# netty/netty

Measured on AMD Instinct MI355X. Metric: GiB/s device-resident Snappy encode+decode, 64 KiB chunks, 1/2/4/8 MI355X, higher is better.
Workload: dtype u8; 1 GPU; configs[4]: Snappy encode (+frame CRC32C) then decode + CRC32C verify of 1638400 text-like 64 KiB chunks (100 GiB) split across 1 GPU(s), device-resident; chunk_bytes=65536, global_chunks=1638400, chunks_per_gpu=1638400, parallelism=dp1 (independent chunk shards, no data-path collective)

## Files before the change

### netty_amd/csrc/snappy_decode.hip

```cpp
#include <stddef.h>
#include <stdlib.h>
#include <type_traits>
#include <string.h>
#include <algorithm>
#include <map>
#include <mutex>
#include "nx_common.hpp"
#include "workspace.hpp"
#include "records.hpp"

namespace nx {
namespace dec {

constexpr int kWaves = 12;
#ifndef NX_RING
#define NX_RING 2048
#endif
constexpr int kRing = NX_RING;
constexpr int kStage = 1024;
constexpr int kFB = 512;
constexpr int kPass = 256;
static_assert((kRing & (kRing - 1)) == 0 && kRing >= 3 * kFB + kPass + 2, "ring");
constexpr int32_t kGuardTrip = -99;
constexpr uint32_t kRecCap = 16384;
constexpr int32_t kNeedFused = -1000;
constexpr uint32_t kSubBatch = NX_DEC_MAX_FRAMES;
constexpr uint32_t kFusedMaxFrames = 32768;
constexpr int kDecodeAuto = 0, kDecodeFused = 1, kDecodePair = 2;

constexpr int kTabWords = 4 * 256 + 4 * 256;
constexpr int kTabBytes = kTabWords * 4;

struct WaveLds {
    uint32_t ring[kRing / 4];
    uint32_t tagw[2 * 64 + 2];
    uint32_t scratch[65];
    uint32_t pad[1];
    uint32_t stage[kStage / 4];
};
constexpr uint32_t kStageDw = offsetof(WaveLds, stage) / 4;
static_assert(sizeof(WaveLds) % 16 == 0 && offsetof(WaveLds, stage) % 16 == 0, "keep per-wave LDS 16-byte aligned");
static_assert(2 * (kTabBytes + kWaves * sizeof(WaveLds)) <= 160 * 1024, "two workgroups per CU");

#ifndef NX_EXPAND_STAGE
#define NX_EXPAND_STAGE 0
#endif
constexpr bool kExpandStaged = NX_EXPAND_STAGE != 0;
constexpr size_t kExpandWaveLds = kExpandStaged ? sizeof(WaveLds) : offsetof(WaveLds, stage);
#ifndef NX_EXPAND_WAVES
#define NX_EXPAND_WAVES (NX_EXPAND_STAGE ? 12 : 4)
#endif
constexpr int kExpandWaves = NX_EXPAND_WAVES;
#ifndef NX_EXPAND_MINB
#define NX_EXPAND_MINB (NX_EXPAND_STAGE ? 3 : 8)
#endif
static_assert(kTabBytes + kExpandWaves * kExpandWaveLds <= 160 * 1024 / NX_EXPAND_MINB, "k_expand workgroups per CU");

typedef uint32_t __attribute__((aligned(1))) u32u;
typedef __attribute__((address_space(1))) const uint8_t gu8;
typedef __attribute__((address_space(1))) const u32u gu32u;
typedef unsigned int v4u __attribute__((ext_vector_type(4)));
typedef __attribute__((address_space(1))) const v4u gv4u;

__device__ __forceinline__ uint32_t shift_byte_tab(const uint32_t* __restrict__ S, uint32_t c) {
    return S[c & 0xFF] ^ S[256 + ((c >> 8) & 0xFF)] ^ S[512 + ((c >> 16) & 0xFF)] ^ S[768 + (c >> 24)];
}

__device__ __forceinline__ uint32_t shift_nib_tab(const uint32_t* __restrict__ N, uint32_t c) {
    uint32_t r = 0;
#pragma unroll
    for (int k = 0; k < 8; ++k) r ^= N[k * 16 + ((c >> (4 * k)) & 15u)];
    return r;
}

__device__ __forceinline__ uint32_t raw8(const uint32_t* __restrict__ T, uint32_t w0, uint32_t w1) {
    uint32_t c = w0;
    c = T[3 * 256 + (c & 0xFF)] ^ T[2 * 256 + ((c >> 8) & 0xFF)] ^ T[1 * 256 + ((c >> 16) & 0xFF)] ^ T[c >> 24];
    c ^= w1;
    c = T[3 * 256 + (c & 0xFF)] ^ T[2 * 256 + ((c >> 8) & 0xFF)] ^ T[1 * 256 + ((c >> 16) & 0xFF)] ^ T[c >> 24];
    return c;
}

__device__ __forceinline__ uint32_t uni(uint32_t v) { return (uint32_t)__builtin_amdgcn_readfirstlane((int)v); }

__device__ __forceinline__ void wave_sync() {
    __builtin_amdgcn_fence(__ATOMIC_RELEASE, "wavefront");
    __builtin_amdgcn_wave_barrier();
    __builtin_amdgcn_fence(__ATOMIC_ACQUIRE, "wavefront");
}

__device__ __forceinline__ uint64_t lanemask_le(int lane) { return lane == 63 ? ~0ull : ((2ull << lane) - 1ull); }

__device__ __forceinline__ uint32_t incl_scan(uint32_t v) {
    v += (uint32_t)__builtin_amdgcn_update_dpp(0, (int)v, 0x111, 0xf, 0xf, false);
    v += (uint32_t)__builtin_amdgcn_update_dpp(0, (int)v, 0x112, 0xf, 0xf, false);
    v += (uint32_t)__builtin_amdgcn_update_dpp(0, (int)v, 0x114, 0xf, 0xf, false);
    v += (uint32_t)__builtin_amdgcn_update_dpp(0, (int)v, 0x118, 0xf, 0xf, false);
    v += (uint32_t)__builtin_amdgcn_update_dpp(0, (int)v, 0x142, 0xa, 0xf, false);
    v += (uint32_t)__builtin_amdgcn_update_dpp(0, (int)v, 0x143, 0xc, 0xf, false);
    return v;
}

__device__ __forceinline__ uint32_t incl_max_scan(uint32_t v) {
    v = max(v, (uint32_t)__builtin_amdgcn_update_dpp(0, (int)v, 0x111, 0xf, 0xf, false));
    v = max(v, (uint32_t)__builtin_amdgcn_update_dpp(0, (int)v, 0x112, 0xf, 0xf, false));
    v = max(v, (uint32_t)__builtin_amdgcn_update_dpp(0, (int)v, 0x114, 0xf, 0xf, false));
    v = max(v, (uint32_t)__builtin_amdgcn_update_dpp(0, (int)v, 0x118, 0xf, 0xf, false));
    v = max(v, (uint32_t)__builtin_amdgcn_update_dpp(0, (int)v, 0x142, 0xa, 0xf, false));
    v = max(v, (uint32_t)__builtin_amdgcn_update_dpp(0, (int)v, 0x143, 0xc, 0xf, false));
    return v;
}

__device__ __forceinline__ uint32_t g_ld32u(const uint8_t* p) { return *(gu32u*)(p); }
__device__ __forceinline__ uint32_t g_ld8(const uint8_t* p) { return *(gu8*)(p); }

struct Frame {
    const uint8_t* src;
    uint32_t in_len;
    uint8_t* dst;
    uint32_t cap;
};

struct FrameIO {
    WaveLds& L;
    const uint8_t* __restrict__ src;
    uint8_t* __restrict__ dst;
    const uint32_t* __restrict__ sT;
    const uint32_t* __restrict__ sSH;
    uint32_t in_len;
    uint32_t a;
    uint32_t aend;
    uint32_t sbase;
    uint2 pf;
    uint32_t flushed;
    uint32_t acc;
    bool dst8, do_crc;
    int lane;

    __device__ __forceinline__ FrameIO(WaveLds& L_, const Frame& f, const uint32_t* T, const uint32_t* SH, bool crc, int ln)
        : L(L_), src(f.src), dst(f.dst), sT(T), sSH(SH), in_len(uni(f.in_len)), sbase(0), pf(make_uint2(0, 0)), flushed(0),
          acc(0), do_crc(crc), lane(ln) {
        a = (uint32_t)((uintptr_t)src & 7u);
        aend = a + in_len;
        dst8 = (((uintptr_t)dst) & 7u) == 0;
    }
    __device__ __forceinline__ uint2 load8(uint32_t apos) const {
        return apos < aend ? *reinterpret_cast<const uint2*>(src - a + apos) : make_uint2(0, 0);
    }
    __device__ __forceinline__ void put8(uint32_t apos, uint2 v) {
        *reinterpret_cast<uint2*>(&reinterpret_cast<uint8_t*>(L.stage)[apos & (kStage - 1)]) = v;
    }
    __device__ __forceinline__ void prime(uint32_t wa) {
        sbase = wa & ~511u;
        put8(sbase + 8u * lane, load8(sbase + 8u * lane));
        put8(sbase + 512u + 8u * lane, load8(sbase + 512u + 8u * lane));
        pf = load8(sbase + 1024u + 8u * lane);
    }
    __device__ __forceinline__ void advance(uint32_t wa) {
        while (wa >= sbase + 512u) {
            if (wa >= sbase + 1536u) {
                prime(wa);
                break;
            }
            put8(sbase + 1024u + 8u * lane, pf);
            sbase += 512u;
            pf = load8(sbase + 1024u + 8u * lane);
        }
    }
    __device__ __forceinline__ void flush_to(uint32_t limit) {
        const uint8_t* ring8 = reinterpret_cast<const uint8_t*>(L.ring);
        while (flushed + (uint32_t)kFB <= limit) {
            wave_sync();
            asm volatile("s_waitcnt vmcnt(1)" ::: "memory");
            const uint2 d = *reinterpret_cast<const uint2*>(&ring8[(flushed + 8u * lane) & (kRing - 1)]);
            uint8_t* o = dst + flushed + 8u * lane;
            if (dst8) {
                *reinterpret_cast<uint2*>(o) = d;
            } else {
#pragma unroll
                for (int i = 0; i < 8; ++i) o[i] = (uint8_t)((i < 4 ? d.x : d.y) >> (8 * (i & 3)));
            }
            if (do_crc) acc = shift_byte_tab(sSH, acc) ^ raw8(sT, (flushed == 0u && lane == 0) ? ~d.x : d.x, d.y);
            flushed += (uint32_t)kFB;
        }
    }
    __device__ uint32_t finish(uint32_t O, const uint32_t* __restrict__ gNS) {
        const uint8_t* ring8 = reinterpret_cast<const uint8_t*>(L.ring);
        flush_to(O);
        wave_sync();
        const uint32_t rem = O - flushed;
        const uint32_t k = rem >> 3;
        asm volatile("s_waitcnt vmcnt(0)" ::: "memory");
        {
            const uint32_t b0 = 8u * lane, b1 = b0 + 8u < rem ? b0 + 8u : rem;
            for (uint32_t i = b0; i < b1; ++i) dst[flushed + i] = ring8[(flushed + i) & (kRing - 1)];
        }
        uint32_t crc = 0;
        if (do_crc) {
            auto fold = [&](uint32_t v) {
#pragma unroll
                for (int j = 0; j < 6; ++j) {
                    const uint32_t other = __shfl_xor(v, 1 << j);
                    const bool is_lo = ((lane >> j) & 1) == 0;
                    v = shift_nib_tab(gNS + j * 128, is_lo ? v : other) ^ (is_lo ? other : v);
                }
                return v;
            };
            uint32_t R = fold(acc);
            uint32_t c2 = 0;
            if ((uint32_t)lane >= 64u - k) {
                const uint32_t pos = flushed + 8u * ((uint32_t)lane - (64u - k));
                const uint2 d = *reinterpret_cast<const uint2*>(&ring8[pos & (kRing - 1)]);
                c2 = raw8(sT, pos == 0u ? ~d.x : d.x, d.y);
            }
            c2 = fold(c2);
#pragma unroll
            for (int j = 0; j < 6; ++j)
                if ((k >> j) & 1u) R = shift_nib_tab(gNS + j * 128, R);
            R ^= c2;
            if (O < 8u) R = 0xFFFFFFFFu;
            for (uint32_t i = flushed + 8u * k; i < O; ++i) R = (R >> 8) ^ sT[(R ^ ring8[i & (kRing - 1)]) & 0xFFu];
            crc = ~R;
        }
        return crc;
    }
};

struct Window {
    uint32_t rec, pdone, O;
};

__device__ bool expand_tags(FrameIO& io, uint32_t lds_base, uint32_t O, uint32_t E, bool prod, uint64_t prodm, uint32_t ostart,
                            uint32_t xv, int lane, uint32_t P0s = 0u, bool last = true, Window* nw = nullptr, uint32_t* rn = nullptr,
                            bool staged = true) {
    WaveLds& L = io.L;
    const uint8_t* ring8 = reinterpret_cast<const uint8_t*>(L.ring);
    const uint32_t* lds32 = L.ring;
    const uint32_t rank = __builtin_amdgcn_mbcnt_hi((uint32_t)(prodm >> 32), __builtin_amdgcn_mbcnt_lo((uint32_t)prodm, 0u));
    if (prod) *reinterpret_cast<uint2*>(&L.tagw[2 * rank]) = make_uint2(ostart, xv);
    if (lane == 0) L.tagw[2 * (uint32_t)__popcll(prodm)] = E;
    const uint64_t unal = __ballot(prod && (ostart & 3u) != 0u);
    const uint64_t first_bit = prodm & (~prodm + 1ull);
    const uint32_t pbase = (ostart >> 2) - (O >> 2) + (uint32_t)__popcll(unal & lanemask_le(lane) & ~first_bit);
    const uint32_t Ptot = ((E + 3u) >> 2) - (O >> 2) + (uint32_t)__popcll(unal & ~first_bit);
    uint32_t rc = 0;
    uint32_t pbc = 0;
    const uint32_t Pend = last ? Ptot : P0s + ((Ptot - P0s) & ~63u);
    uint32_t* const marks = L.scratch;
    uint32_t P0 = P0s;
    if (P0 >= Pend) {
        if (rn) asm volatile("" : "+v"(*rn));
    } else do {
        L.scratch[lane] = 0u;
        wave_sync();
        {
            const uint32_t rel = pbase - P0;
            const bool in_pass = prod && rel < 64u;
            marks[in_pass ? rel : 64u] = ((rank + 1u) << 6) | (rel & 63u);
        }
        wave_sync();
        const uint32_t mk = incl_max_scan(L.scratch[lane]);
        const uint32_t P = P0 + lane;
        const bool valid = P < Ptot;
        uint32_t r = mk ? (mk >> 6) - 1u : rc;
        const uint32_t k = mk ? (uint32_t)lane - (mk & 63u) : P - pbc;
        r = valid ? r : 0u;
        {
            const uint32_t mlast = uni((uint32_t)__builtin_amdgcn_readlane((int)mk, 63));
            if (mlast) {
                rc = (mlast >> 6) - 1u;
                pbc = P0 + (mlast & 63u);
            }
        }
        const uint32_t tstart = L.tagw[2 * r], tx = L.tagw[2 * r + 1], tend = L.tagw[2 * r + 2];
        const uint32_t A = ((tstart >> 2) + k) << 2;
        const uint32_t x0 = A > tstart ? A : tstart;
        const uint32_t x1 = (A + 4u) < tend ? A + 4u : tend;
        const uint32_t last = (Ptot - P0) < 64u ? (Ptot - P0 - 1u) : 63u;
        const uint32_t ps = uni((uint32_t)__builtin_amdgcn_readlane((int)x0, 0));
        const uint32_t pe = uni((uint32_t)__builtin_amdgcn_readlane((int)x1, (int)last));

        const bool lit = (tx & 0x80000000u) == 0u;
        const uint32_t xo = tx & 0x7FFFFFFFu;
        const uint32_t tlen = tend - tstart;
        const bool overlap = !lit && xo < tlen;
        const uint32_t pin = xo + (x0 - tstart);
        const uint32_t sp = lit ? pin + io.a : x0 - xo;
        const bool gl = lit ? (!staged || (sp - io.sbase) > (uint32_t)(kStage - 8))
                            : (!overlap && pe > (uint32_t)kRing && sp < pe - (uint32_t)kRing);
        const uint32_t lbase = lit && staged ? kStageDw : 0u;
        const uint32_t lmask = lit && staged ? (uint32_t)(kStage / 4 - 1) : (uint32_t)(kRing / 4 - 1);
        const uint32_t nbytes = x1 - x0;
        const uint32_t sh = 8u * (x0 & 3u);
        const uint32_t bmask = (nbytes >= 4u ? 0xFFFFFFFFu : ((1u << (8u * nbytes)) - 1u)) << sh;
        const uint32_t waddr = lds_base + 4u * ((x0 >> 2) & (kRing / 4 - 1));
        uint32_t gval;
        uint32_t gsh = 0;
        uint32_t gtiny = 0;
        const bool gld = valid && gl;
        const bool tiny = io.in_len < 4u;
        if (__ballot(gld)) {
            const bool tail = lit && pin + 4u > io.in_len;
            const uint8_t* ga = !lit ? io.dst + sp : io.src + (tail ? io.in_len - 4u : pin);
            if (gld && !tiny) gval = g_ld32u(ga);
            gsh = tail ? 8u * (pin + 4u - io.in_len) : 0u;
            if (tiny && __ballot(gld)) {
                if (gld) {
#pragma unroll
                    for (uint32_t i = 0; i < 4; ++i)
                        if (pin + i < io.in_len) gtiny |= g_ld8(io.src + pin + i) << (8 * i);
                }
            }
        }
        const uint32_t psal = ps & ~3u;
        const uint32_t dhi = overlap ? tstart : sp + nbytes;
        const bool dep = valid && !lit && !gl && dhi > ps;
        uint64_t need = 0;
        const uint64_t depm = __ballot(dep);
        if (depm) {
            wave_sync();
            {
                const uint32_t mm = valid ? bmask : 0u;
                const uint32_t maddr = lds_base + (uint32_t)offsetof(WaveLds, scratch) + (valid ? 4u * ((x0 >> 2) - (psal >> 2)) : 0u);
                asm volatile("ds_mskor_b32 %0, %1, %2" ::"v"(maddr), "v"(mm), "v"(((uint32_t)lane * 0x01010101u) & mm) : "memory");
            }
            wave_sync();
            const uint32_t lo0 = overlap ? tstart - xo : sp;
            const uint8_t* M8 = reinterpret_cast<const uint8_t*>(L.scratch);
            const uint32_t lo = lo0 > ps ? lo0 : ps;
            const uint32_t pa = M8[dep ? lo - psal : 0u], pb = M8[dep ? dhi - 1u - psal : 0u];
            const uint64_t nm = (pb >= 63u ? ~0ull : ((2ull << pb) - 1ull)) & ~((1ull << (pa & 63u)) - 1ull);
            need = dep ? nm : 0ull;
        }
        const bool has_ov = __ballot(valid && overlap) != 0ull;
        uint32_t ova = 0, ovb = 0;
        if (has_ov) {
            const uint32_t n0 = x0 - tstart;
            const uint32_t inv = (uint32_t)(__builtin_amdgcn_rcpf((float)xo) * 65536.0f) + 1u;
            const uint32_t m0 = n0 - xo * ((n0 * inv) >> 16);
            const uint32_t q = tstart - xo;
            uint32_t ad[4];
            uint32_t mi = m0;
#pragma unroll
            for (uint32_t i = 0; i < 4; ++i) {
                if (i) mi = mi + 1u == xo ? 0u : mi + 1u;
                ad[i] = (q + mi) & (kRing - 1);
            }
            ova = ad[0] | (ad[1] << 16);
            ovb = ad[2] | (ad[3] << 16);
        }
        const uint32_t w = sp >> 2;
        const uint32_t ra0 = lbase + (w & lmask), ra1 = lbase + ((w + 1u) & lmask);
        uint64_t pending = depm;
        const uint64_t validm = last >= 63u ? ~0ull : ((2ull << last) - 1ull);
        uint64_t readym = validm & ~depm;
        for (int round = 0;; ++round) {
            uint32_t lo = lds32[ra0];
            uint32_t hi = lds32[ra1];
            asm volatile("" : "+v"(lo), "+v"(hi));
            uint32_t val = gl ? (tiny ? gtiny : gval >> gsh) : __builtin_amdgcn_alignbyte(hi, lo, sp & 3u);
            if (has_ov) {
                const uint32_t ov = (uint32_t)ring8[ova & 0xFFFFu] | ((uint32_t)ring8[ova >> 16] << 8) |
                                    ((uint32_t)ring8[ovb & 0xFFFFu] << 16) | ((uint32_t)ring8[ovb >> 16] << 24);
                val = overlap ? ov : val;
            }
            uint32_t m;
            asm volatile("v_cndmask_b32_e64 %0, 0, %1, %2" : "=v"(m) : "v"(bmask), "s"(readym));
            asm volatile("ds_mskor_b32 %0, %1, %2" ::"v"(waddr), "v"(m), "v"((val << sh) & m) : "memory");
            if (!pending || round >= 64) break;
            readym = __ballot((need & pending) == 0ull) & validm;
            pending &= ~readym;
        }
        if (pending) return false;
        if (rn) asm volatile("" : "+v"(*rn));
        io.flush_to(pe);
    } while ((P0 += 64u) < Pend);
    if (!last) {
        if (Pend == Ptot) {
            nw->rec = (uint32_t)__popcll(prodm);
            nw->pdone = 0u;
            nw->O = E;
        } else {
            const uint32_t idx = (uint32_t)__popcll(__ballot(prod && pbase <= Pend)) - 1u;
            nw->rec = idx;
            nw->pdone = Pend - uni((uint32_t)__builtin_amdgcn_readlane((int)pbase, (int)idx));
            nw->O = uni((uint32_t)__builtin_amdgcn_readlane((int)ostart, (int)idx));
        }
    }
    return true;
}

__device__ __forceinline__ void write_result(int lane, uint32_t crc, int32_t st, bool check, uint32_t expect, uint32_t O,
                                             uint32_t consumed, uint32_t* out_len_p, uint32_t* consumed_p, int32_t* status_p,
                                             uint32_t* crc_p) {
    if (lane == 0) {
        const uint32_t m = mask_checksum(crc);
        if (st == NX_OK && check && m != expect) st = NX_ERR_SNAPPY_CRC_MISMATCH;
        *out_len_p = O;
        if (consumed_p) *consumed_p = consumed;
        *status_p = st;
        if (crc_p) *crc_p = m;
    }
}

__device__ void decode_frame_fused(WaveLds& L, uint32_t lds_base, const Frame& f, const uint32_t* __restrict__ sT,
                                   const uint32_t* __restrict__ sSH, const uint32_t* __restrict__ gNS, bool do_crc, uint32_t expect,
                                   bool check, uint32_t* out_len_p, uint32_t* consumed_p, int32_t* status_p, uint32_t* crc_p,
                                   int lane) {
    FrameIO io(L, f, sT, sSH, do_crc, lane);
    const uint8_t* __restrict__ src = f.src;
    const uint32_t in_len = io.in_len;
    const uint32_t cap = uni(f.cap < (1u << 24) ? f.cap : (1u << 24));
    int32_t st = NX_OK;
    uint32_t consumed = 0;
    uint32_t O = 0;

    uint32_t W = 0;
    bool go = false;
    if (in_len > 0) {
        uint32_t ulen = 0;
        int bi = 0;
        bool complete = false;
        while (W < in_len) {
            const uint32_t cur = uni(src[W++]);
            ulen |= (cur & 0x7fu) << (bi++ * 7);
            if ((cur & 0x80u) == 0) {
                complete = true;
                break;
            }
            if (bi >= 4) {
                st = NX_ERR_SNAPPY_PREAMBLE_TOO_LONG;
                break;
            }
        }
        if (st == NX_OK && complete && ulen != 0) {
            if (ulen > cap) st = NX_ERR_SNAPPY_OUTPUT_OVERFLOW; else go = true;
        }
        consumed = W;
    }
    W = uni(W);
    if (go) io.prime(W + io.a);

    bool stop = !go;
    uint32_t windows = 0;
    while (!stop && W < in_len) {
        if (++windows > in_len + 2) {
            st = kGuardTrip;
            break;
        }
        io.advance(W + io.a);
        wave_sync();
        const uint32_t p = W + lane;
        const uint32_t avail = p < in_len ? in_len - p : 0u;
        uint64_t v;
        {
            const uint32_t pa = p + io.a;
            const uint32_t w0 = L.stage[(pa >> 2) & (kStage / 4 - 1)];
            const uint32_t w1 = L.stage[((pa >> 2) + 1) & (kStage / 4 - 1)];
            v = (((uint64_t)w1 << 32) | w0) >> (8 * (pa & 3u));
            if (avail < 5) v &= (1ull << (8 * avail)) - 1ull;
        }
        const uint32_t b0 = (uint32_t)v & 0xFFu;
        const uint32_t type = b0 & 3u;
        const uint32_t ops = (uint32_t)(v >> 8);
        const uint32_t code = b0 >> 2;
        const uint32_t nb = code >= 60u ? code - 59u : 0u;
        const uint32_t hdr = 1u + nb;
        const uint32_t field = nb == 0 ? 0u : (nb == 4 ? ops : (ops & ((1u << (8 * nb)) - 1u)));
        const uint32_t lj = nb == 0 ? code + 1u : field + 1u;
        const bool lneg = nb == 4 && (int32_t)lj < 0;
        const bool lhdr_nei = avail < hdr;
        const bool l_nei = lhdr_nei || (!lneg && (avail - hdr) < lj);
        const uint32_t csize = type == 1u ? 2u : (type == 2u ? 3u : 5u);
        const uint32_t colen = type == 1u ? 4u + ((b0 >> 2) & 7u) : 1u + (b0 >> 2);
        const uint32_t coff = type == 1u ? (((b0 & 0xe0u) << 3) | (ops & 0xFFu)) : (type == 2u ? (ops & 0xFFFFu) : ops);
        const bool c_nei = avail < csize;
        const bool is_copy = type != 0u;
        const bool nei = is_copy ? c_nei : l_nei;
        int32_t err = 0;
        if (is_copy) {
            if (!c_nei && coff == 0u) err = NX_ERR_SNAPPY_OFFSET_ZERO;
            else if (!c_nei && type == 3u && (int32_t)coff < 0) err = NX_ERR_SNAPPY_OFFSET_NEGATIVE;
        } else if (!lhdr_nei && lneg) {
            err = NX_ERR_SNAPPY_LITERAL_LEN_INVALID;
        }
        uint32_t size;
        uint32_t olen;
        if (is_copy) {
            size = csize;
            olen = colen;
        } else {
            const uint64_t sz = (uint64_t)hdr + (lneg ? 0ull : (uint64_t)lj);
            size = sz > 0x7FFFFFFFull ? 0x7FFFFFFFu : (uint32_t)sz;
            olen = lneg ? 0u : (lj > cap ? cap + 1u : lj);
        }
        const uint32_t xv = is_copy ? (0x80000000u | (coff & 0x7FFFFFFFu)) : ((p + hdr) & 0x7FFFFFFFu);
        const uint32_t nxt = (uint32_t)lane + size;

        const uint32_t lim = uni((in_len - W) < 64u ? (in_len - W) : 64u);
        uint32_t Jk[6];
        Jk[0] = (uint32_t)lane >= lim ? (uint32_t)lane : (nxt < 64u ? nxt : 64u);
#pragma unroll
        for (int k = 1; k < 6; ++k) {
            const uint32_t prev = Jk[k - 1];
            const uint32_t g = (uint32_t)__shfl((int)prev, (int)(prev & 63u));
            Jk[k] = prev >= 64u ? 64u : g;
        }
        uint32_t pos = 0;
#pragma unroll
        for (int k = 0; k < 6; ++k) {
            const uint32_t g = (uint32_t)__shfl((int)Jk[k], (int)(pos & 63u));
            if (((uint32_t)lane >> k) & 1u) pos = pos >= 64u ? 64u : g;
        }
        const bool tvm = pos < lim;
        const uint32_t T = (uint32_t)__popcll(__ballot(tvm));
        const uint32_t lastpos = uni((uint32_t)__builtin_amdgcn_readlane((int)pos, (int)(T - 1)));
        const uint32_t exitrel = uni((uint32_t)__builtin_amdgcn_readlane((int)nxt, (int)lastpos));
        L.scratch[lane] = 0;
        wave_sync();
        if (tvm) L.scratch[pos] = 1u;
        wave_sync();
        const bool tv = L.scratch[lane] != 0u;

        const uint32_t mylen = tv ? olen : 0u;
        const uint32_t incl = incl_scan(mylen);
        const uint32_t ostart = O + incl - mylen;
        if (tv && is_copy && !nei && err == 0 && (coff & 0x7FFFFFFFu) > ostart) err = NX_ERR_SNAPPY_OFFSET_BEYOND;
        if (tv && !nei && err == 0 && (uint64_t)ostart + olen > cap) err = NX_ERR_SNAPPY_OUTPUT_OVERFLOW;
        const uint64_t badm = __ballot(tv && (nei || err != 0));
        const uint32_t Wnext = uni(W + exitrel);
        uint32_t fb = 64;
        uint32_t E;
        if (badm) {
            fb = (uint32_t)(__ffsll((long long)badm) - 1);
            const int32_t e = __builtin_amdgcn_readlane(err, (int)fb);
            if (e != 0) {
                st = e;
                consumed = W + uni((uint32_t)__builtin_amdgcn_readlane((int)nxt, (int)fb));
            } else {
                consumed = W + fb + 1;
            }
            stop = true;
            E = uni((uint32_t)__builtin_amdgcn_readlane((int)ostart, (int)fb));
        } else {
            consumed = Wnext < in_len ? Wnext : in_len;
            E = O + uni((uint32_t)__builtin_amdgcn_readlane((int)incl, 63));
        }
        const bool prod = tv && (uint32_t)lane < fb && olen > 0;
        const uint64_t prodm = __ballot(prod);
        if (prodm && !expand_tags(io, lds_base, O, E, prod, prodm, ostart, xv, lane)) {
            st = kGuardTrip + 2;
            break;
        }
        O = E;
        W = Wnext;
    }
    const uint32_t crc = io.finish(O, gNS);
    write_result(lane, crc, st, check, expect, O, consumed, out_len_p, consumed_p, status_p, crc_p);
}

struct WaveSetup {
    uint32_t* sT;
    uint32_t* sSH;
    WaveLds* L;
    uint32_t lds_base;
    uint32_t wave;
};
__device__ __forceinline__ WaveSetup wave_setup(uint8_t* smem, const CrcTables* __restrict__ tabs, bool do_crc,
                                                size_t wave_lds = sizeof(WaveLds)) {
    WaveSetup s;
    s.sT = reinterpret_cast<uint32_t*>(smem);
    s.sSH = s.sT + 4 * 256;
    if (do_crc) {
        for (int i = threadIdx.x; i < 4 * 256; i += blockDim.x) s.sT[i] = (&tabs->T8[0][0])[i];
        for (int i = threadIdx.x; i < 4 * 256; i += blockDim.x) s.sSH[i] = (&tabs->SH[5][0][0])[i];
    }
    __syncthreads();
    s.wave = uni(threadIdx.x >> 6);
    s.L = reinterpret_cast<WaveLds*>(smem + kTabBytes + s.wave * wave_lds);
    s.lds_base = (uint32_t)(uintptr_t)s.L;
    return s;
}

__global__ void __launch_bounds__(kWaves * 64, 6)
    k_decode_fused(const uint8_t* __restrict__ in, const uint64_t* __restrict__ in_off, const uint32_t* __restrict__ in_len,
                   uint8_t* __restrict__ out, const uint64_t* __restrict__ out_off, const uint32_t* __restrict__ out_cap,
// ... 98 lines not shown
            x[0].y = w[33];
            x[0].z = w[34];
            x[0].w = w[35];
        } else if (B != 0u) {
            x[0] = *(const gv4u*)(origin + (B - 16u <= last ? B - 16u : last));
        } else {
            x[0] = v4u{0u, 0u, 0u, 0u};
        }
        lb = B;
#pragma unroll
        for (uint32_t k = 0; k < 9; ++k) {
            w[4 * k] = x[k].x;
            w[4 * k + 1] = x[k].y;
            w[4 * k + 2] = x[k].z;
            w[4 * k + 3] = x[k].w;
        }
    }
    __device__ __forceinline__ uint64_t get8(uint32_t p) const {
        const uint32_t off = p + pad + 16u - lb;
        const uint32_t i = off >> 2, s = off & 3u;
        const uint32_t d0 = w[i], d1 = w[i + 1], d2 = w[i + 2];
        return (uint64_t)__builtin_amdgcn_alignbyte(d1, d0, s) | ((uint64_t)__builtin_amdgcn_alignbyte(d2, d1, s) << 32);
    }
};
#ifndef NX_PARSE_LINE
#define NX_PARSE_LINE 0
#endif
#ifndef NX_PARSE_DEFER
#define NX_PARSE_DEFER 0
#endif
#ifndef NX_PARSE_RELOAD_K
#define NX_PARSE_RELOAD_K 16
#endif


template <uint32_t QR, bool DEFER = false>
struct RecWriterT {
    static_assert(QR == 4 || QR == 8 || QR == 16, "record row");
    static constexpr uint32_t kStride = QR == 16 ? 20u : QR + 1u;
    static constexpr uint32_t kV = QR / 4;
    uint4* slot;
    uint32_t* q;
    uint32_t n;
    v4u p0, p1, p2, p3;
    uint32_t pend_at;
    __device__ __forceinline__ RecWriterT(uint4* s, uint32_t* row) : slot(s), q(row), n(0), pend_at(0xFFFFFFFFu) {}
    __device__ __forceinline__ v4u row(uint32_t k) const {
        if constexpr (QR == 16) {
            return reinterpret_cast<const v4u*>(q)[k];
        } else {
            return v4u{q[4 * k], q[4 * k + 1], q[4 * k + 2], q[4 * k + 3]};
        }
    }
    __device__ __forceinline__ void drain() {
        if constexpr (DEFER) {
            if (pend_at != 0xFFFFFFFFu) {
                v4u* d = reinterpret_cast<v4u*>(slot + (pend_at >> 2));
                d[0] = p0;
                if constexpr (kV > 1) d[1] = p1;
                if constexpr (kV > 2) {
                    d[2] = p2;
                    d[3] = p3;
                }
                pend_at = 0xFFFFFFFFu;
            }
        }
    }
    __device__ __forceinline__ bool put(uint32_t r) {
        if constexpr (!DEFER) {
            const bool ok = n < kRecCap;
            q[n & (QR - 1u)] = r;
            if (ok & ((n & (QR - 1u)) == QR - 1u)) {
                v4u* d = reinterpret_cast<v4u*>(slot + ((n - (QR - 1u)) >> 2));
#pragma unroll
                for (uint32_t k = 0; k < kV; ++k) d[k] = row(k);
            }
            n += ok ? 1u : 0u;
            return ok;
        }
        if (n >= kRecCap) return false;
        drain();
        q[n & (QR - 1u)] = r;
        if ((n & (QR - 1u)) == QR - 1u) {
            if constexpr (DEFER) {
                p0 = row(0);
                if constexpr (kV > 1) p1 = row(1);
                if constexpr (kV > 2) {
                    p2 = row(2);
                    p3 = row(3);
                }
                pend_at = n - (QR - 1u);
            } else {
                v4u* d = reinterpret_cast<v4u*>(slot + ((n - (QR - 1u)) >> 2));
#pragma unroll
                for (uint32_t k = 0; k < kV; ++k) d[k] = row(k);
            }
        }
        ++n;
        return true;
    }
    __device__ __forceinline__ void finish() {
        drain();
        const uint32_t k = n & (QR - 1u);
        if (k) {
            v4u* d = reinterpret_cast<v4u*>(slot + ((n - k) >> 2));
#pragma unroll
            for (uint32_t j = 0; j < kV; ++j)
                if (4u * j < k) d[j] = row(j);
        }
    }
};
using RecWriter = RecWriterT<16>;
constexpr int kQDw = (int)RecWriter::kStride;
#ifndef NX_PARSE_QR
#define NX_PARSE_QR 16
#endif
#ifndef NX_PARSE_NB
#define NX_PARSE_NB 4
#endif
using ParseRec = RecWriterT<NX_PARSE_QR, NX_PARSE_DEFER != 0>;
using ParseBurst = BurstWinT<NX_PARSE_NB>;
using ParseWin = std::conditional_t<NX_PARSE_LINE != 0, BurstWinLine, ParseBurst>;

template <int K, class Has, class Step>
__device__ __forceinline__ void burst_steps(const bool& run, Has has, Step step) {
    if constexpr (K > 0) {
        for (;;) {
            const bool act = run & has();
            if (!__any(act) || __popcll(__ballot(run & !act)) >= K) break;
            if (act) step();
        }
    } else {
        while (run & has()) step();
    }
}
#ifndef NX_ALT_RELOAD_K
#define NX_ALT_RELOAD_K 0
#endif

__global__ void __launch_bounds__(kParseBlock) k_parse(const uint8_t* __restrict__ in, const uint64_t* __restrict__ in_off,
                                                       const uint32_t* __restrict__ in_len_a, const uint32_t* __restrict__ out_cap,
                                                       uint32_t* __restrict__ rec, uint32_t* __restrict__ nrec,
                                                       uint32_t* __restrict__ out_len, uint32_t* __restrict__ consumed_a,
                                                       int32_t* __restrict__ status, uint32_t n, uint32_t* __restrict__ need_fused) {
    __shared__ uint32_t wins[kParseBlock * ParseWin::kStride + 4];
    __shared__ __attribute__((aligned(16))) uint32_t recq[kParseBlock * ParseRec::kStride];
    const uint32_t c = blockIdx.x * blockDim.x + threadIdx.x;
    if (c >= n) return;
    const uint32_t in_len = in_len_a[c];
    uint32_t cap = out_cap ? out_cap[c] : 65536u;
    cap = cap < (1u << 24) ? cap : (1u << 24);
    if (in_len >= (1u << 25)) {
        status[c] = kNeedFused;
        if (need_fused) *need_fused = 1u;
        return;
    }
    ParseWin win;
    win.init(in + in_off[c], in_len, &wins[threadIdx.x * ParseWin::kStride]);
    ParseRec rw(reinterpret_cast<uint4*>(rec + (size_t)c * kRecCap), &recq[threadIdx.x * ParseRec::kStride]);
    uint32_t ip = 0, op = 0;
    int32_t st = NX_OK;
    bool run = false;
    if (in_len > 0) {
        win.load(0);
        const uint64_t v = win.get8(0);
        uint32_t ulen = 0;
        int bi = 0;
        bool complete = false;
        while (ip < in_len) {
            const uint32_t cur = (uint32_t)(v >> (8 * ip)) & 0xFFu;
            ++ip;
            ulen |= (cur & 0x7fu) << (bi++ * 7);
            if ((cur & 0x80u) == 0) {
                complete = true;
                break;
            }
            if (bi >= 4) {
                st = NX_ERR_SNAPPY_PREAMBLE_TOO_LONG;
                break;
            }
        }
        if (st == NX_OK && complete && ulen != 0) {
            if (ulen > cap) st = NX_ERR_SNAPPY_OUTPUT_OVERFLOW; else run = true;
        }
    }
    auto step = [&]() {
        const uint64_t v = win.get8(ip);
        const uint32_t tag = (uint32_t)v & 0xFFu;
        const uint32_t ops = (uint32_t)(v >> 8);
        const uint32_t after_tag = ip + 1u;
        const uint32_t avail = in_len - after_tag;
        const uint32_t type = tag & 3u;
        const bool isl = type == 0u;
        const uint32_t code = tag >> 2;
        const uint32_t nb = (isl && code >= 60u) ? code - 59u : 0u;
        const uint32_t fmask = nb >= 4u ? 0xFFFFFFFFu : ((1u << (8u * nb)) - 1u);
        const uint32_t lj = nb == 0u ? code + 1u : (ops & fmask) + 1u;
        const uint32_t csize = type == 1u ? 1u : (type == 2u ? 2u : 4u);
        const uint32_t clen = type == 1u ? 4u + (code & 7u) : 1u + code;
        const uint32_t coff = type == 1u ? (((tag & 0xe0u) << 3) | (ops & 0xFFu)) : (type == 2u ? (ops & 0xFFFFu) : ops);
        const uint32_t hdr = isl ? nb : csize;
        const uint32_t dpos = after_tag + hdr;
        const bool lneg = isl && (int32_t)lj < 0;
        const bool nei = avail < hdr || (isl && !lneg && in_len - dpos < lj);
        const uint32_t len = isl ? lj : clen;
        const bool bad = (uint32_t)(isl ? lneg : coff - 1u >= op) | (uint32_t)(len > cap - op);
        if (nei | bad) {
            const int32_t cerr = coff == 0u ? NX_ERR_SNAPPY_OFFSET_ZERO
                                            : ((int32_t)coff < 0 ? NX_ERR_SNAPPY_OFFSET_NEGATIVE : (coff > op ? NX_ERR_SNAPPY_OFFSET_BEYOND : 0));
            const int32_t terr = isl ? (lneg ? NX_ERR_SNAPPY_LITERAL_LEN_INVALID : 0) : cerr;
            ip = nei ? after_tag : dpos;
            st = nei ? NX_OK : (terr != 0 ? terr : NX_ERR_SNAPPY_OUTPUT_OVERFLOW);
            run = false;
            return;
        }
        const uint32_t m0 = lj < 64u ? lj : 64u;
        const uint32_t r = isl ? (((m0 - 1u) << 25) | dpos) : (0x80000000u | ((clen - 1u) << 25) | coff);
        bool fit = (isl && lj == 0u) || rw.put(r);
        if (isl && lj > 64u) {
            for (uint32_t k = 64u; k < lj && fit; k += 64u) {
                const uint32_t m = lj - k < 64u ? lj - k : 64u;
                fit = rw.put(((m - 1u) << 25) | (dpos + k));
            }
        }
        if (!fit) {
            st = kNeedFused;
            run = false;
            return;
        }
        ip = dpos + (isl ? lj : 0u);
        op += len;
        run = ip < in_len;
    };
    for (;;) {
        run = run && ip < in_len;
        if (!__any(run)) break;
        if (run && !win.has(ip)) win.load(ip);
        burst_steps<NX_PARSE_RELOAD_K>(run, [&] { return win.has(ip); }, step);
    }
    if (st == kNeedFused) {
        status[c] = kNeedFused;
        if (need_fused) *need_fused = 1u;
        return;
    }
    rw.finish();
    nrec[c] = rw.n;
    out_len[c] = op;
    if (consumed_a) consumed_a[c] = ip;
    status[c] = st;
}

#ifdef NX_EXPAND_NUM_SGPR
#define NX_EXPAND_SGPR_ATTR __attribute__((amdgpu_num_sgpr(NX_EXPAND_NUM_SGPR)))
#else
#define NX_EXPAND_SGPR_ATTR
#endif
__global__ void __launch_bounds__(kExpandWaves * 64, NX_EXPAND_MINB) NX_EXPAND_SGPR_ATTR
    k_expand(const uint8_t* __restrict__ in, const uint64_t* __restrict__ in_off, const uint32_t* __restrict__ in_len,
             uint8_t* __restrict__ out, const uint64_t* __restrict__ out_off, const uint32_t* __restrict__ rec,
             const uint32_t* __restrict__ nrec, uint32_t* __restrict__ out_len, int32_t* __restrict__ status,
             const uint32_t* __restrict__ expect, uint32_t* __restrict__ crc_out, uint32_t n, const CrcTables* __restrict__ tabs) {
    extern __shared__ __attribute__((aligned(16))) uint8_t smem[];
    const bool do_crc = (expect != nullptr) || (crc_out != nullptr);
    const WaveSetup s = wave_setup(smem, tabs, do_crc, kExpandWaveLds);
    const int lane = threadIdx.x & 63;
    const uint32_t nw = gridDim.x * kExpandWaves;
    for (uint32_t c = blockIdx.x * kExpandWaves + s.wave; c < n; c += nw) {
        int32_t st = (int32_t)uni((uint32_t)status[c]);
        if (st == kNeedFused) continue;
        const uint32_t N = uni(nrec[c]);
        const uint32_t Ofin = uni(out_len[c]);
        Frame f{in + in_off[c], in_len[c], out + out_off[c], 0u};
        FrameIO io(*s.L, f, s.sT, s.sSH, do_crc, lane);
        const uint32_t* __restrict__ R = rec + (size_t)c * kRecCap;
        uint32_t O = 0;
        uint32_t pdone = 0;
        bool primed = false;
        uint32_t r = (uint32_t)lane < N ? R[lane] : 0u;
        asm volatile("" : "+v"(r));
        for (uint32_t b = 0; b < N;) {
            const bool valid = b + (uint32_t)lane < N;
            const bool isc = (r >> 31) != 0u;
            const uint32_t len = valid ? ((r >> 25) & 63u) + 1u : 0u;
            asm volatile("" ::"v"(len) : "memory");
            uint32_t rnext = b + 64u + (uint32_t)lane < N ? R[b + 64u + lane] : 0u;
            const uint32_t x = r & 0x1FFFFFFu;
            const uint32_t incl = incl_scan(len);
            const uint32_t ostart = O + incl - len;
            const uint32_t E = O + uni((uint32_t)__builtin_amdgcn_readlane((int)incl, 63));
            const uint64_t litm = kExpandStaged ? __ballot(valid && !isc) : 0ull;
            if (litm) {
                const uint32_t w = uni((uint32_t)__builtin_amdgcn_readlane((int)x, __ffsll((long long)litm) - 1));
                if (!primed) {
                    io.prime(w + io.a);
                    primed = true;
                } else {
                    io.advance(w + io.a);
                }
                wave_sync();
            }
            const uint32_t xv = isc ? (0x80000000u | x) : x;
            const bool last = b + 64u >= N;
            Window nw{0u, 0u, 0u};
            if (!expand_tags(io, s.lds_base, O, E, valid, __ballot(valid), ostart, xv, lane, pdone, last, &nw, &rnext, kExpandStaged)) {
                st = kGuardTrip + 2;
                break;
            }
            if (last) {
                O = E;
                break;
            }
            const uint32_t src = (uint32_t)lane + nw.rec;
            const uint32_t from_r = (uint32_t)__shfl((int)r, (int)(src & 63u));
            const uint32_t from_n = (uint32_t)__shfl((int)rnext, (int)(src & 63u));
            r = src < 64u ? from_r : from_n;
            b += nw.rec;
            pdone = nw.pdone;
            O = nw.O;
        }
        if (st == kGuardTrip + 2) O = Ofin;
        const uint32_t crc = io.finish(O, &tabs->NS[0][0][0]);
        write_result(lane, crc, st, expect != nullptr, expect ? expect[c] : 0u, O, 0u, &out_len[c], nullptr, &status[c],
                     crc_out ? &crc_out[c] : nullptr);
    }
}





__device__ __forceinline__ bool put_copy(RecWriter& rw, uint32_t len, uint32_t dist) {
    bool fit = true;
    for (uint32_t k = 0; k < len && fit; k += 64u) {
        const uint32_t m = len - k < 64u ? len - k : 64u;
        fit = rw.put(0x80000000u | ((m - 1u) << 25) | dist);
    }
    return fit;
}

template <class Win>
__device__ __forceinline__ uint32_t win_byte(Win& win, uint32_t p) {
    if (!win.has(p)) win.load(p);
    return (uint32_t)win.get8(p) & 0xFFu;
}

__global__ void __launch_bounds__(kParseBlock) k_parse_lz4(const uint8_t* __restrict__ in, const uint64_t* __restrict__ in_off,
                                                           const uint32_t* __restrict__ in_len_a, const uint32_t* __restrict__ want_a,
                                                           uint32_t* __restrict__ rec, uint32_t* __restrict__ nrec,
                                                           uint32_t* __restrict__ out_len, int32_t* __restrict__ status, uint32_t n) {
    __shared__ uint32_t wins[kParseBlock * kWinDw + 4];
    __shared__ __attribute__((aligned(16))) uint32_t recq[kParseBlock * kQDw];
    const uint32_t c = blockIdx.x * blockDim.x + threadIdx.x;
    if (c >= n) return;
    const uint32_t in_len = in_len_a[c];
    const uint32_t want = want_a[c];
    if (in_len >= (1u << 25) || want > 65536u) {
        status[c] = kNeedFused;
        return;
    }
    BurstWin win;
    win.init(in + in_off[c], in_len, &wins[threadIdx.x * kWinDw]);
    RecWriter rw(reinterpret_cast<uint4*>(rec + (size_t)c * kRecCap), &recq[threadIdx.x * kQDw]);
    uint32_t ip = 0, op = 0;
    int32_t st = NX_OK;
    bool fit = true;
    for (;;) {
        if (ip >= in_len) {
            st = NX_ERR_LZ4_MALFORMED;
            break;
        }
        const uint32_t token = win_byte(win, ip++);
        uint32_t lit = token >> 4;
        if (lit == 15u) {
            uint32_t b = 255u;
            while (b == 255u && ip < in_len) {
                b = win_byte(win, ip++);
                lit += b;
            }
            if (b == 255u) {
                st = NX_ERR_LZ4_MALFORMED;
                break;
            }
        }
        if (lit > in_len - ip || lit > want - op) {
            st = NX_ERR_LZ4_MALFORMED;
            break;
        }
        for (uint32_t k = 0; k < lit && fit; k += 64u) {
            const uint32_t m = lit - k < 64u ? lit - k : 64u;
            fit = rw.put(((m - 1u) << 25) | (ip + k));
        }
        if (!fit) break;
        ip += lit;
        op += lit;
        if (ip == in_len) break;
        if (in_len - ip < 2u) {
            st = NX_ERR_LZ4_MALFORMED;
            break;
        }
        const uint32_t off = win_byte(win, ip) | (win_byte(win, ip + 1u) << 8);
        ip += 2u;
        if (off == 0u || off > op) {
            st = NX_ERR_LZ4_MALFORMED;
            break;
        }
        uint32_t ml = token & 15u;
        if (ml == 15u) {
            uint32_t b = 255u;
            while (b == 255u && ip < in_len) {
                b = win_byte(win, ip++);
                ml += b;
            }
            if (b == 255u) {
                st = NX_ERR_LZ4_MALFORMED;
                break;
            }
        }
        ml += 4u;
        if (ml > want - op) {
            st = NX_ERR_LZ4_MALFORMED;
            break;
        }
        for (uint32_t k = 0; k < ml && fit; k += 64u) {
            const uint32_t m = ml - k < 64u ? ml - k : 64u;
            fit = rw.put(0x80000000u | ((m - 1u) << 25) | off);
        }
        if (!fit) break;
        op += ml;
    }
    if (!fit) {
        status[c] = kNeedFused;
        return;
    }
    if (st == NX_OK && op != want) st = NX_ERR_LZ4_MALFORMED;
    rw.finish();
    nrec[c] = rw.n;
    out_len[c] = op;
    status[c] = st;
}

__global__ void __launch_bounds__(256) k_lz4_serial(const uint8_t* __restrict__ in, const uint64_t* __restrict__ in_off,
                                                    const uint32_t* __restrict__ in_len_a, const uint32_t* __restrict__ want_a,
                                                    uint8_t* __restrict__ out, const uint64_t* __restrict__ out_off,
                                                    int32_t* __restrict__ status, uint32_t n) {
    const uint32_t c = blockIdx.x * blockDim.x + threadIdx.x;
    if (c >= n || status[c] != kNeedFused) return;
    const uint8_t* s = in + in_off[c];
    uint8_t* d = out + out_off[c];
    const uint64_t in_len = in_len_a[c], want = want_a[c];
    uint64_t ip = 0, op = 0;
    int32_t st = NX_OK;
    for (;;) {
        if (ip >= in_len) {
            st = NX_ERR_LZ4_MALFORMED;
            break;
        }
        const uint32_t token = s[ip++];
        uint64_t lit = token >> 4;
        if (lit == 15u) {
            uint32_t b = 255u;
            while (b == 255u && ip < in_len) {
                b = s[ip++];
                lit += b;
            }
            if (b == 255u) {
                st = NX_ERR_LZ4_MALFORMED;
                break;
            }
        }
        if (lit > in_len - ip || lit > want - op) {
            st = NX_ERR_LZ4_MALFORMED;
            break;
        }
        for (uint64_t k = 0; k < lit; ++k) d[op + k] = s[ip + k];
        ip += lit;
        op += lit;
        if (ip == in_len) break;
        if (in_len - ip < 2u) {
            st = NX_ERR_LZ4_MALFORMED;
            break;
        }
        const uint64_t off = (uint64_t)s[ip] | ((uint64_t)s[ip + 1] << 8);
        ip += 2;
        if (off == 0u || off > op) {
            st = NX_ERR_LZ4_MALFORMED;
            break;
        }
        uint64_t ml = token & 15u;
        if (ml == 15u) {
            uint32_t b = 255u;
            while (b == 255u && ip < in_len) {
                b = s[ip++];
                ml += b;
            }
            if (b == 255u) {
                st = NX_ERR_LZ4_MALFORMED;
                break;
            }
        }
        ml += 4u;
        if (ml > want - op) {
            st = NX_ERR_LZ4_MALFORMED;
            break;
        }
        for (uint64_t k = 0; k < ml; ++k) d[op + k] = d[op + k - off];
        op += ml;
    }
    if (st == NX_OK && op != want) st = NX_ERR_LZ4_MALFORMED;
    status[c] = st;
}


#ifndef FLZ_WIN_BLOCKS
#define FLZ_WIN_BLOCKS 4
#endif
__global__ void __launch_bounds__(kParseBlock) k_parse_fastlz(const uint8_t* __restrict__ in, const uint64_t* __restrict__ in_off,
                                                              const uint32_t* __restrict__ in_len_a, const uint32_t* __restrict__ avail_a,
                                                              const uint32_t* __restrict__ lim_a, uint32_t* __restrict__ rec,
                                                              uint32_t* __restrict__ nrec, uint32_t* __restrict__ out_len,
                                                              int32_t* __restrict__ status, uint32_t n) {
    using Win = BurstWinT<FLZ_WIN_BLOCKS>;
    __shared__ uint32_t wins[kParseBlock * Win::kStride + 4];
    __shared__ __attribute__((aligned(16))) uint32_t recq[kParseBlock * kQDw];
    const uint32_t c = blockIdx.x * blockDim.x + threadIdx.x;
    if (c >= n) return;
    const uint32_t in_len = in_len_a[c];
    const uint32_t lim = lim_a[c];
    if (in_len < 1u || in_len >= (1u << 24) || lim >= (1u << 24) || (avail_a && avail_a[c] < in_len)) {
        status[c] = kNeedSerial;
        return;
    }
    Win win;
    win.init(in + in_off[c], in_len, &wins[threadIdx.x * Win::kStride]);
    RecWriter rw(reinterpret_cast<uint4*>(rec + (size_t)c * kRecCap), &recq[threadIdx.x * kQDw]);
    win.load(0);
    const uint32_t b0 = (uint32_t)win.get8(0) & 0xFFu;
    const uint32_t level = (b0 >> 5) + 1u;
    const uint32_t k0 = (b0 & 31u) + 1u;
    bool ok = (level == 1u || level == 2u) && k0 <= lim && 1u + k0 <= in_len && rw.put(((k0 - 1u) << 25) | 1u);
    uint32_t ip = 1u + k0, op = k0;
    bool run = ok && ip < in_len;
    for (;;) {
        if (!__any(run)) break;
        if (run && !win.has(ip)) win.load(ip);
        burst_steps<NX_ALT_RELOAD_K>(run, [&] { return win.has(ip); }, [&] {
            const uint64_t v = win.get8(ip);
            const uint32_t ctrl = (uint32_t)v & 0xFFu;
            uint32_t adv, len, dist;
            bool put_ok;
            if (ctrl < 32u) {
                const uint32_t k = ctrl + 1u;
                if (op + k > lim || ip + 1u + k > in_len) {
                    ok = false;
                    run = false;
                    return;
                }
                put_ok = rw.put(((k - 1u) << 25) | (ip + 1u));
                adv = 1u + k;
                len = k;
            } else {
                len = (ctrl >> 5) - 1u;
                const uint32_t ofs = (ctrl & 31u) << 8;
                uint32_t p = 1u;
                if (len == 6u && level == 2u && ((uint32_t)(v >> 8) & 0xFFu) == 255u) {
                    uint32_t code = 255u;
                    while (code == 255u) {
                        if (ip + p >= in_len) break;
                        code = win_byte(win, ip + p);
                        ++p;
                        len += code;
                    }
                    if (code == 255u || ip + p + 2u >= in_len + 0u) {
                        ok = false;
                        run = false;
                        return;
                    }
                    const uint32_t cd = win_byte(win, ip + p);
                    ++p;
                    dist = ofs + cd + 1u;
                    if (cd == 255u && ofs == (31u << 8)) {
                        dist = ((win_byte(win, ip + p) << 8) | win_byte(win, ip + p + 1u)) + 8192u;
                        p += 2u;
                    }
                } else {
                    if (len == 6u) {
                        len += (uint32_t)(v >> 8) & 0xFFu;
                        p = 2u;
                    }
                    const uint32_t code = (uint32_t)(v >> (8u * p)) & 0xFFu;
                    ++p;
                    dist = ofs + code + 1u;
                    if (level == 2u && code == 255u && ofs == (31u << 8)) {
                        const uint32_t hi = (uint32_t)(v >> (8u * p)) & 0xFFu, lo = (uint32_t)(v >> (8u * p + 8u)) & 0xFFu;
                        dist = ((hi << 8) | lo) + 8192u;
                        p += 2u;
                    }
                }
                if (ip + p > in_len || op + len + 3u > lim || dist > op) {
                    ok = false;
                    run = false;
                    return;
                }
                len += 3u;
                put_ok = put_copy(rw, len, dist);
                adv = p;
            }
            if (!put_ok) {
// ... 280 lines not shown
```

Measured before the change: 52.61 GiB/s.

## Replace per-pass LDS max-scan piece-to-tag mapping with a precomputed piece-start bitmap

In the windowed expand path, each tag's starting piece index is set once in a per-wave LDS bitmap with ds_or, before the pass loop. Each 64-piece pass then finds its owning tag with mbcnt over a 64-bit slice of that bitmap, which replaces the per-pass scratch clear, two wave syncs and the inclusive max-scan. The tag's unaligned-slip count is packed into the upper bits of the tag word so each piece's address can be rebuilt directly. This adds LDS per wave and cuts the usable offset field to 25 bits, and it may bring correctness risks near window edges.

```diff
diff --git a/netty_amd/csrc/snappy_decode.hip b/netty_amd/csrc/snappy_decode.hip
--- a/netty_amd/csrc/snappy_decode.hip
+++ b/netty_amd/csrc/snappy_decode.hip
@@ -31,13 +31,18 @@
 constexpr int kTabWords = 4 * 256 + 4 * 256;
 constexpr int kTabBytes = kTabWords * 4;
 
+constexpr uint32_t kWinPieces = 64 * 17;
+constexpr uint32_t kWinPieceDw = (kWinPieces / 32 + 3) & ~3u;
+
 struct WaveLds {
     uint32_t ring[kRing / 4];
     uint32_t tagw[2 * 64 + 2];
     uint32_t scratch[65];
     uint32_t pad[1];
+    uint32_t pstart[kWinPieceDw];
     uint32_t stage[kStage / 4];
 };
+static_assert(offsetof(WaveLds, pstart) % 8 == 0, "a pass reads its 64 piece-start bits as one qword");
 constexpr uint32_t kStageDw = offsetof(WaveLds, stage) / 4;
 static_assert(sizeof(WaveLds) % 16 == 0 && offsetof(WaveLds, stage) % 16 == 0, "keep per-wave LDS 16-byte aligned");
 static_assert(2 * (kTabBytes + kWaves * sizeof(WaveLds)) <= 160 * 1024, "two workgroups per CU");
@@ -230,6 +235,7 @@
     uint32_t rec, pdone, O;
 };
 
+template <bool kRecWin = false>
 __device__ bool expand_tags(FrameIO& io, uint32_t lds_base, uint32_t O, uint32_t E, bool prod, uint64_t prodm, uint32_t ostart,
                             uint32_t xv, int lane, uint32_t P0s = 0u, bool last = true, Window* nw = nullptr, uint32_t* rn = nullptr,
                             bool staged = true) {
@@ -237,12 +243,24 @@
     const uint8_t* ring8 = reinterpret_cast<const uint8_t*>(L.ring);
     const uint32_t* lds32 = L.ring;
     const uint32_t rank = __builtin_amdgcn_mbcnt_hi((uint32_t)(prodm >> 32), __builtin_amdgcn_mbcnt_lo((uint32_t)prodm, 0u));
-    if (prod) *reinterpret_cast<uint2*>(&L.tagw[2 * rank]) = make_uint2(ostart, xv);
-    if (lane == 0) L.tagw[2 * (uint32_t)__popcll(prodm)] = E;
     const uint64_t unal = __ballot(prod && (ostart & 3u) != 0u);
     const uint64_t first_bit = prodm & (~prodm + 1ull);
-    const uint32_t pbase = (ostart >> 2) - (O >> 2) + (uint32_t)__popcll(unal & lanemask_le(lane) & ~first_bit);
+    const uint32_t slip = (uint32_t)__popcll(unal & lanemask_le(lane) & ~first_bit);
+    const uint32_t pbase = (ostart >> 2) - (O >> 2) + slip;
     const uint32_t Ptot = ((E + 3u) >> 2) - (O >> 2) + (uint32_t)__popcll(unal & ~first_bit);
+    if (prod) *reinterpret_cast<uint2*>(&L.tagw[2 * rank]) = make_uint2(ostart, kRecWin ? xv | (slip << 25) : xv);
+    if (lane == 0) L.tagw[2 * (uint32_t)__popcll(prodm)] = E;
+    uint32_t cnt = 0;
+    if constexpr (kRecWin) {
+        if ((uint32_t)lane < kWinPieceDw) L.pstart[lane] = 0u;
+        wave_sync();
+        const uint32_t rel = pbase - P0s;
+        const bool in_win = prod && rel < kWinPieces;
+        const uint32_t baddr = lds_base + (uint32_t)offsetof(WaveLds, pstart) + (in_win ? 4u * (rel >> 5) : 0u);
+        asm volatile("ds_or_b32 %0, %1" ::"v"(baddr), "v"(in_win ? 1u << (rel & 31u) : 0u) : "memory");
+        wave_sync();
+        cnt = (uint32_t)__popcll(__ballot(prod && pbase < P0s));
+    }
     uint32_t rc = 0;
     uint32_t pbc = 0;
     const uint32_t Pend = last ? Ptot : P0s + ((Ptot - P0s) & ~63u);
@@ -251,21 +269,28 @@
     if (P0 >= Pend) {
         if (rn) asm volatile("" : "+v"(*rn));
     } else do {
-        L.scratch[lane] = 0u;
-        wave_sync();
-        {
-            const uint32_t rel = pbase - P0;
-            const bool in_pass = prod && rel < 64u;
-            marks[in_pass ? rel : 64u] = ((rank + 1u) << 6) | (rel & 63u);
-        }
-        wave_sync();
-        const uint32_t mk = incl_max_scan(L.scratch[lane]);
         const uint32_t P = P0 + lane;
         const bool valid = P < Ptot;
-        uint32_t r = mk ? (mk >> 6) - 1u : rc;
-        const uint32_t k = mk ? (uint32_t)lane - (mk & 63u) : P - pbc;
-        r = valid ? r : 0u;
-        {
+        uint32_t r, k = 0;
+        if constexpr (kRecWin) {
+            const uint2 mq = *reinterpret_cast<const uint2*>(&L.pstart[(P0 - P0s) >> 5]);
+            const uint32_t mlo = uni(mq.x), mhi = uni(mq.y);
+            const uint64_t above = (((uint64_t)mhi << 32) | mlo) >> 1;
+            r = __builtin_amdgcn_mbcnt_hi((uint32_t)(above >> 32), __builtin_amdgcn_mbcnt_lo((uint32_t)above, cnt + (mlo & 1u) - 1u));
+            cnt += (uint32_t)__popc(mlo) + (uint32_t)__popc(mhi);
+        } else {
+            L.scratch[lane] = 0u;
+            wave_sync();
+            {
+                const uint32_t rel = pbase - P0;
+                const bool in_pass = prod && rel < 64u;
+                marks[in_pass ? rel : 64u] = ((rank + 1u) << 6) | (rel & 63u);
+            }
+            wave_sync();
+            const uint32_t mk = incl_max_scan(L.scratch[lane]);
+            r = mk ? (mk >> 6) - 1u : rc;
+            k = mk ? (uint32_t)lane - (mk & 63u) : P - pbc;
+            r = valid ? r : 0u;
             const uint32_t mlast = uni((uint32_t)__builtin_amdgcn_readlane((int)mk, 63));
             if (mlast) {
                 rc = (mlast >> 6) - 1u;
@@ -273,7 +298,7 @@
             }
         }
         const uint32_t tstart = L.tagw[2 * r], tx = L.tagw[2 * r + 1], tend = L.tagw[2 * r + 2];
-        const uint32_t A = ((tstart >> 2) + k) << 2;
+        const uint32_t A = (kRecWin ? P + (O >> 2) - ((tx >> 25) & 63u) : (tstart >> 2) + k) << 2;
         const uint32_t x0 = A > tstart ? A : tstart;
         const uint32_t x1 = (A + 4u) < tend ? A + 4u : tend;
         const uint32_t last = (Ptot - P0) < 64u ? (Ptot - P0 - 1u) : 63u;
@@ -281,7 +306,7 @@
         const uint32_t pe = uni((uint32_t)__builtin_amdgcn_readlane((int)x1, (int)last));
 
         const bool lit = (tx & 0x80000000u) == 0u;
-        const uint32_t xo = tx & 0x7FFFFFFFu;
+        const uint32_t xo = tx & (kRecWin ? 0x1FFFFFFu : 0x7FFFFFFFu);
         const uint32_t tlen = tend - tstart;
         const bool overlap = !lit && xo < tlen;
         const uint32_t pin = xo + (x0 - tstart);
@@ -986,7 +1011,7 @@
             const uint32_t xv = isc ? (0x80000000u | x) : x;
             const bool last = b + 64u >= N;
             Window nw{0u, 0u, 0u};
-            if (!expand_tags(io, s.lds_base, O, E, valid, __ballot(valid), ostart, xv, lane, pdone, last, &nw, &rnext, kExpandStaged)) {
+            if (!expand_tags<true>(io, s.lds_base, O, E, valid, __ballot(valid), ostart, xv, lane, pdone, last, &nw, &rnext, kExpandStaged)) {
                 st = kGuardTrip + 2;
                 break;
             }
```

New measurement: 50.57 GiB/s. 0.961x the previous value.
